# AKASH2907/pi-consistency-activity-detection

Measured on AMD Instinct MI355X. Metric: train clips/sec (bs=8, 16×224×224, I3D+caps+bv cons) at 1/2/4/8 GPU, higher is better.
Workload: dtype f32 (fp32 operands and fp32 accumulation everywhere; 33 of the 79 conv / input-gradient launches and the 3x3x3 / 1x1x1 weight gradients multiply on the bf16 matrix cores: every fp32 operand as the exact sum of 3 bf16 terms, 6 products on v_mfma_f32_32x32x16_bf16, hi / lo fp32 accumulators -- error v

## Files before the change

pi-consistency-activity-detection_amd/csrc/elementwise.hip:

```cpp
#include "common.h"
#include <stdlib.h>

namespace {

constexpr int FIN_RL = 16;
constexpr int FIN_CL = 16;
constexpr int FIN_T = FIN_RL * FIN_CL;

template <typename TP>
__device__ __forceinline__ void partial_colsum(const TP* __restrict__ part, int npg, int C, int c, int rl,
                                               double (*sh)[FIN_RL][FIN_CL], int cl, double& s, double& s2) {
    double a[4] = {0, 0, 0, 0}, b[4] = {0, 0, 0, 0};
    if (c < C) {
        int i = rl;
        for (; i + 3 * FIN_RL < npg; i += 4 * FIN_RL) {
            TP x[4], y[4];
#pragma unroll
            for (int u = 0; u < 4; ++u) { const TP* q = part + (size_t)(i + u * FIN_RL) * 2 * C + c; x[u] = q[0]; y[u] = q[C]; }
#pragma unroll
            for (int u = 0; u < 4; ++u) { a[u] += (double)x[u]; b[u] += (double)y[u]; }
        }
        for (; i < npg; i += FIN_RL) { const TP* q = part + (size_t)i * 2 * C + c; a[0] += (double)q[0]; b[0] += (double)q[C]; }
    }
    sh[0][rl][cl] = (a[0] + a[1]) + (a[2] + a[3]); sh[1][rl][cl] = (b[0] + b[1]) + (b[2] + b[3]);
// ... 525 lines not shown
                if (to > hi[0]) break;
                const int a = t + d.padf[0] - to * ST;
                uchar4 ix[MH * MW];
                f32x4 v[MH * MW];
#pragma unroll
                for (int jh = 0; jh < MH; ++jh)
#pragma unroll
                    for (int jw = 0; jw < MW; ++jw) {
                        const int ho = min(lo[1] + jh, d.Ho - 1), wo = min(lo[2] + jw, d.Wo - 1);
                        const size_t op = (size_t)((n * d.To + to) * d.Ho + ho) * d.Wo + wo;
                        ix[jh * MW + jw] = *(const uchar4*)(am + op * d.C + c);
                        v[jh * MW + jw] = *(const f32x4*)(dy + op * d.ldo + c);
                    }
#pragma unroll
                for (int jh = 0; jh < MH; ++jh)
#pragma unroll
                    for (int jw = 0; jw < MW; ++jw) {
                        const int ho = lo[1] + jh, wo = lo[2] + jw;
                        const int tap = (ho <= hi[1] && wo <= hi[2]) ? (a * KH + (h + d.padf[1] - ho * SH)) * KW + (w + d.padf[2] - wo * SW) : 256;
                        const uchar4 q = ix[jh * MW + jw];
                        const f32x4 u = v[jh * MW + jw];
                        if (q.x == tap) g[0] += u[0];
                        if (q.y == tap) g[1] += u[1];
                        if (q.z == tap) g[2] += u[2];
                        if (q.w == tap) g[3] += u[3];
                    }
            }
        }
        if (accum) g += old;
        *(f32x4*)o = g;
    }
}

__global__ __launch_bounds__(256) void chscale_kernel(const float* __restrict__ x, int ldx, const float* __restrict__ sc, int64_t pos_per_n,
                                                      int C4, int64_t total4, float* __restrict__ y, int ldy, int accum) {
    const int C = C4 * 4;
    for (int64_t idx = (int64_t)blockIdx.x * 256 + threadIdx.x; idx < total4; idx += (int64_t)gridDim.x * 256) {
        const size_t row = (unsigned)idx / (unsigned)C4;
        const int c = (int)((unsigned)idx - (unsigned)row * C4) * 4;
        const size_t n = (unsigned)row / (unsigned)pos_per_n;
        const f32x4 v = *(const f32x4*)(x + row * ldx + c), s = *(const f32x4*)(sc + n * C + c);
        f32x4 o = v * s;
        float* q = y + row * ldy + c;
        if (accum) o += *(const f32x4*)q;
        *(f32x4*)q = o;
    }
}

template <typename T>
__global__ __launch_bounds__(256) void to_ndhwc_kernel(const T* __restrict__ src, int N, int C, int64_t thw, int W, int Cpad, int flipw,
                                                       float* __restrict__ dst) {
    const int64_t total = (int64_t)N * thw;
    for (int64_t idx = (int64_t)blockIdx.x * 256 + threadIdx.x; idx < total; idx += (int64_t)gridDim.x * 256) {
        const int64_t n = idx / thw, pos = idx - n * thw;
        int64_t sp = pos;
        if (flipw) { const int w = (int)(pos % W); sp = pos - w + (W - 1 - w); }
        if (Cpad == 4) {
            f32x4 v;
#pragma unroll
            for (int c = 0; c < 4; ++c) v[c] = c < C ? (float)src[(n * C + c) * thw + sp] : 0.f;
            *(f32x4*)(dst + idx * 4) = v;
            continue;
        }
        for (int c = 0; c < Cpad; ++c)
            dst[idx * Cpad + c] = c < C ? (float)src[(n * C + c) * thw + sp] : 0.f;
    }
// ... 50 lines not shown
        if (i < J.tr) {
            const int r = r0 + i, c = c0 + c4;
            f32x4 sum = {0.f, 0.f, 0.f, 0.f};
            if (r < J.R && c < J.Cc) {
                const f32x4* q = (const f32x4*)(J.src + (size_t)b * J.sbs + (size_t)r * J.sld + c);
                const size_t st4 = (size_t)J.sst / 4;
                int k = 0;
                for (; k + 16 <= J.nsl; k += 16) {
                    f32x4 t[16];
#pragma unroll
                    for (int u = 0; u < 16; ++u) t[u] = q[(size_t)(k + u) * st4];
#pragma unroll
                    for (int u = 0; u < 16; ++u) sum += t[u];
                }
                for (; k + 4 <= J.nsl; k += 4) {
                    f32x4 t[4];
#pragma unroll
                    for (int u = 0; u < 4; ++u) t[u] = q[(size_t)(k + u) * st4];
#pragma unroll
                    for (int u = 0; u < 4; ++u) sum += t[u];
                }
                for (; k < J.nsl; ++k) sum += q[(size_t)k * st4];
            }
            tile[i][c4] = sum[0]; tile[i][c4 + 1] = sum[1]; tile[i][c4 + 2] = sum[2]; tile[i][c4 + 3] = sum[3];
        }
    }
    __syncthreads();
    for (int i = ty; i < 32; i += 8) {
        const int c = c0 + i, r = r0 + tx;
        if (tx < J.tr && c < J.Cc && r < J.R) {
            float* o = J.dst + (size_t)b * J.dbs + (size_t)c * J.dld + r;
            *o = (J.accum ? *o : 0.f) + tile[tx][i];
        }
    }
}

template <int GROUP>
__global__ __launch_bounds__(256) void slices_fold_kernel(float* __restrict__ ws, int64_t image4, int nslices, int64_t total) {
    for (int64_t idx = (int64_t)blockIdx.x * 256 + threadIdx.x; idx < total; idx += (int64_t)gridDim.x * 256) {
        const int64_t e = idx % image4; const int g = (int)(idx / image4);
        float4* base = (float4*)ws + (int64_t)g * GROUP * image4 + e;
        const int n = min(GROUP, nslices - g * GROUP);
        float4 t[GROUP];
#pragma unroll
        for (int k = 0; k < GROUP; ++k) if (k < n) t[k] = base[(int64_t)k * image4];
        float4 sum = t[0];
#pragma unroll
        for (int k = 1; k < GROUP; ++k) if (k < n) { sum.x += t[k].x; sum.y += t[k].y; sum.z += t[k].z; sum.w += t[k].w; }
        base[0] = sum;
    }
}

__global__ __launch_bounds__(256) void fill_kernel(float* p, int64_t n, float v) {
    for (int64_t i = (int64_t)blockIdx.x * 256 + threadIdx.x; i < n; i += (int64_t)gridDim.x * 256) p[i] = v;
}
__global__ __launch_bounds__(256) void axpy_kernel(float* y, const float* x, int64_t n, float a) {
    for (int64_t i = (int64_t)blockIdx.x * 256 + threadIdx.x; i < n; i += (int64_t)gridDim.x * 256) y[i] += a * x[i];
}

__global__ __launch_bounds__(256) void adam_kernel(float* __restrict__ p, const float* __restrict__ g, float* __restrict__ m, float* __restrict__ v,
                                                   int64_t n, float lr_bc1, float b1, float b2, float omb1, float omb2, float eps, float inv_sqrt_bc2,
                                                   float gscale) {
    for (int64_t i = (int64_t)blockIdx.x * 256 + threadIdx.x; i < n; i += (int64_t)gridDim.x * 256) {
        const float gi = g[i] * gscale;
        const float mi = b1 * m[i] + omb1 * gi;
        const float vi = b2 * v[i] + omb2 * gi * gi;
// ... 2 lines not shown
    }
}

__global__ __launch_bounds__(256) void col2im_kernel(const float* __restrict__ cols, int N, int Ho, int Wo, int KH, int KW, int C4,
                                                     float* __restrict__ dx, int lddx, int accum, int64_t total4) {
    const int Hi = Ho + KH - 1, Wi = Wo + KW - 1, C = C4 * 4;
    const size_t ldc = (size_t)KH * KW * C;
    for (int64_t idx = (int64_t)blockIdx.x * 256 + threadIdx.x; idx < total4; idx += (int64_t)gridDim.x * 256) {
        int64_t pos = idx / C4;
        const int c = (int)(idx - pos * C4) * 4;
        const int64_t ipos = pos;
        const int w = (int)(pos % Wi); pos /= Wi;
        const int h = (int)(pos % Hi); const int n = (int)(pos / Hi);
        f32x4 acc = {0.f, 0.f, 0.f, 0.f};
        const int b0 = max(0, h - (Ho - 1)), b1 = min(KH - 1, h), c0 = max(0, w - (Wo - 1)), c1 = min(KW - 1, w);
        for (int b = b0; b <= b1; ++b)
            for (int cc = c0; cc <= c1; ++cc) {
                const size_t op = (size_t)((n * Ho + (h - b)) * Wo + (w - cc));
                acc += *(const f32x4*)(cols + op * ldc + (size_t)(b * KW + cc) * C + c);
            }
        float* o = dx + ipos * lddx + c;
        if (accum) acc += *(const f32x4*)o;
        *(f32x4*)o = acc;
    }
}

inline int grid_for(int64_t n, int per_thread = 1) {
    int64_t b = (n + 256ll * per_thread - 1) / (256ll * per_thread);
    if (b > 256 * 16) b = 256 * 16;
    if (b < 1) b = 1;
    return (int)b;
}
inline int pool_blocks(int64_t total4) { return total4 > POOL_ITEMS ? (int)((total4 + POOL_ITEMS - 1) / POOL_ITEMS) : 1; }
inline int pool_form(const pc_pool_desc* d) {
    const auto is = [](const int32_t* v, int a, int b, int c) { return v[0] == a && v[1] == b && v[2] == c; };
    if (is(d->k, 1, 3, 3) && is(d->s, 1, 2, 2)) return 1;
    if (is(d->k, 3, 3, 3) && is(d->s, 2, 1, 1)) return 2;
    if (is(d->k, 3, 3, 3) && is(d->s, 1, 1, 1)) return 3;
    return 0;
}
inline double pc_decimal_of_float(float x) {
    char buf[40];
    for (int prec = 1; prec <= 9; ++prec) {
        snprintf(buf, sizeof(buf), "%.*g", prec, (double)x);
        const double d = strtod(buf, nullptr);
        if ((float)d == x) return d;
    }
    return (double)x;
}
inline int64_t red_rows_per_block(int64_t rows) {
    int64_t r = (rows + 1023) / 1024;
    if (r < 32) r = 32;
    return r;
}

}

extern "C" int64_t pc_bn_finalize_ws_floats(int nparts_per_group, int groups, int C) {
    return nparts_per_group >= 512 ? (int64_t)groups * FIN_S * 2 * C * 2 + 2 : 0;
}

extern "C" int pc_bn_finalize_ws(const float* part, int nparts_per_group, int groups, int C, int64_t count_per_group,
                                 const float* gamma, const float* beta, float eps, float momentum, float* running_mean,
                                 float* running_var, float* stat, float* ws, pc_stream s) {
    PC_CHECK_ARG(part && gamma && beta && stat && groups >= 1 && C > 0, "pc_bn_finalize: bad args");
    if (ws && nparts_per_group >= 512) {
// ... 80 lines not shown
    {
        RedP p;
        p.a = dy; p.lda = lddy; p.b = z; p.ldb = ldz;
        p.stat = stat; p.C4 = C / 4; p.rows = rpg; p.rows_per_group = rpg; p.rows_per_block = rpb;
        p.act = relu ? PC_ACT_RELU : PC_ACT_NONE; p.part = part;
        p.a_gs = rpg * lddy; p.b_gs = rpg * ldz; p.stat_gs = 4 * C; p.part_gs = (int64_t)npg * 2 * C;
        hipLaunchKernelGGL(colreduce_kernel, dim3(npg, groups), dim3(256), 0, s, p);
    }
    PC_CHECK_LAUNCH("bn_bwd reduce");
    if (fused) {
        PC_CHECK_ARG(rows * (int64_t)(C / 4) < (1ll << 31), "elementwise kernels index with 32 bits");
        const int cblocks = cdiv(C, FA_CB), rb2 = fa_rows_per_block(rpg, cblocks, groups);
        hipLaunchKernelGGL(bn_bwd_fin_apply_kernel, dim3((unsigned)cdiv(rpg, rb2), cblocks, groups), dim3(256), 0, s, part, npg, groups, C, (double)rpg, dy, lddy, z, ldz,
                           stat, relu, dz, lddz, dgamma, dbeta, accum, (int)rpg, rb2);
        PC_CHECK_LAUNCH("bn_bwd fin_apply");
        return PC_OK;
    }
    hipLaunchKernelGGL(bn_bwd_finalize_kernel, dim3(cdiv(C, FIN_CL)), dim3(FIN_T), 0, s, part, npg, groups, C, (double)rpg, coef, dgamma, dbeta, accum);
    const int64_t total4 = rows * (C / 4);
    PC_CHECK_ARG(total4 < (1ll << 31), "elementwise kernels index with 32 bits: %lld float4 elements", (long long)total4);
    hipLaunchKernelGGL(bn_bwd_apply_kernel, dim3(grid_for(total4, 2)), dim3(256), 0, s, dy, lddy, z, ldz, stat, coef, C / 4, total4, rpg, relu, dz, lddz);
    PC_CHECK_LAUNCH("bn_bwd apply");
    return PC_OK;
}

extern "C" int pc_maxpool_fwd(const pc_pool_desc* d, const float* x, float* y, uint8_t* argmax, pc_stream s) {
    PC_CHECK_ARG(d && x && y && argmax && d->C % 4 == 0 && d->ldi % 4 == 0 && d->ldo % 4 == 0, "pc_maxpool_fwd: bad args");
    PC_CHECK_ARG(d->k[0] * d->k[1] * d->k[2] < 255, "pc_maxpool_fwd: window too large");
    const int64_t npos = (int64_t)d->N * d->To * d->Ho * d->Wo, total4 = npos * (d->C / 4);
    PC_CHECK_ARG(total4 < (1ll << 31), "elementwise kernels index with 32 bits: %lld float4 elements", (long long)total4);
    const int nblk = pool_blocks(total4);
    const unsigned ppb = (unsigned)cdiv(npos, nblk);
#define PC_POOL_FWD(...) hipLaunchKernelGGL((maxpool_fwd_kernel<__VA_ARGS__>), dim3(nblk), dim3(256), 0, (hipStream_t)s, *d, x, y, argmax, (unsigned)npos, ppb)
    switch (pool_form(d)) {
        case 1: PC_POOL_FWD(1, 3, 3, 1, 2, 2); break;
        case 2: PC_POOL_FWD(3, 3, 3, 2, 1, 1); break;
        case 3: PC_POOL_FWD(3, 3, 3, 1, 1, 1); break;
        default: PC_POOL_FWD(0, 0, 0, 0, 0, 0);
    }
#undef PC_POOL_FWD
    PC_CHECK_LAUNCH("maxpool_fwd");
    return PC_OK;
}

extern "C" int pc_maxpool_bwd(const pc_pool_desc* d, const float* dy, const uint8_t* argmax, float* dx, int accum, pc_stream s) {
    PC_CHECK_ARG(d && dy && dx && argmax && d->C % 4 == 0 && d->ldi % 4 == 0 && d->ldo % 4 == 0, "pc_maxpool_bwd: bad args");
    const int64_t npos = (int64_t)d->N * d->Ti * d->Hi * d->Wi, total4 = npos * (d->C / 4);
    PC_CHECK_ARG(total4 < (1ll << 31), "elementwise kernels index with 32 bits: %lld float4 elements", (long long)total4);
    const int nblk = pool_blocks(total4);
    const unsigned ppb = (unsigned)cdiv(npos, nblk);
#define PC_POOL_BWD(...) hipLaunchKernelGGL((maxpool_bwd_kernel<__VA_ARGS__>), dim3(nblk), dim3(256), 0, (hipStream_t)s, *d, dy, argmax, dx, accum, (unsigned)npos, ppb)
    switch (pool_form(d)) {
        case 1: PC_POOL_BWD(1, 3, 3, 1, 2, 2); break;
        case 2: PC_POOL_BWD(3, 3, 3, 2, 1, 1); break;
        case 3: PC_POOL_BWD(3, 3, 3, 1, 1, 1); break;
        default: PC_POOL_BWD(0, 0, 0, 0, 0, 0);
    }
#undef PC_POOL_BWD
    PC_CHECK_LAUNCH("maxpool_bwd");
    return PC_OK;
}

extern "C" int pc_channel_scale(const float* x, int ldx, const float* scale, int N, int64_t pos_per_n, int C, float* y, int ldy,
                                int accum, pc_stream s) {
    PC_CHECK_ARG(x && scale && y && C % 4 == 0 && ldx % 4 == 0 && ldy % 4 == 0, "pc_channel_scale: bad args");
    const int64_t total4 = (int64_t)N * pos_per_n * (C / 4);
    PC_CHECK_ARG(total4 < (1ll << 31), "elementwise kernels index with 32 bits: %lld float4 elements", (long long)total4);
    hipLaunchKernelGGL(chscale_kernel, dim3(grid_for(total4, 2)), dim3(256), 0, (hipStream_t)s, x, ldx, scale, pos_per_n, C / 4, total4, y, ldy, accum);
    PC_CHECK_LAUNCH("channel_scale");
    return PC_OK;
}

extern "C" int64_t pc_act_bwd_ws_floats(int64_t rows, int C) {
    const int64_t rpb = red_rows_per_block(rows);
    return ((rows + rpb - 1) / rpb) * 2 * (int64_t)C + 64;
}

extern "C" int pc_act_bwd(const float* dy, int lddy, const float* y, int ldy, int act, int C, int64_t rows, float* dz, int lddz,
                          float* dbias, int accum, float* ws, pc_stream s_) {
    hipStream_t s = (hipStream_t)s_;
    PC_CHECK_ARG(dy && y && C % 4 == 0 && C <= 1024 && lddy % 4 == 0 && ldy % 4 == 0, "pc_act_bwd: bad args (C=%d)", C);
    const bool write = dz && (act != PC_ACT_NONE || dz != dy);
    const int64_t total4 = rows * (C / 4);
    if (write) {
        PC_CHECK_ARG(lddz % 4 == 0, "pc_act_bwd: lddz");
        PC_CHECK_ARG(total4 < (1ll << 31), "elementwise kernels index with 32 bits: %lld float4 elements", (long long)total4);
    }
    if (dbias) {
        PC_CHECK_ARG(ws, "pc_act_bwd: ws required for dbias");
        const int64_t rpb = red_rows_per_block(rows);
// ... 6 lines not shown
    }
    PC_CHECK_LAUNCH("act_bwd");
    return PC_OK;
}

extern "C" int pc_ncdhw_to_ndhwc(const void* src, int src_is_f64, int N, int C, int64_t thw, int W, int Cpad, int flipw, float* dst, pc_stream s) {
    PC_CHECK_ARG(src && dst && Cpad >= C && W > 0 && thw % W == 0, "pc_ncdhw_to_ndhwc: bad args");
    const int64_t total = (int64_t)N * thw;
    if (src_is_f64) hipLaunchKernelGGL(to_ndhwc_kernel<double>, dim3(grid_for(total)), dim3(256), 0, (hipStream_t)s, (const double*)src, N, C, thw, W, Cpad, flipw, dst);
    else hipLaunchKernelGGL(to_ndhwc_kernel<float>, dim3(grid_for(total)), dim3(256), 0, (hipStream_t)s, (const float*)src, N, C, thw, W, Cpad, flipw, dst);
    PC_CHECK_LAUNCH("to_ndhwc");
    return PC_OK;
}

extern "C" int pc_ndhwc_to_ncdhw(const float* src, int ld, int N, int C, int64_t thw, float* dst, pc_stream s) {
    PC_CHECK_ARG(src && dst, "pc_ndhwc_to_ncdhw: null");
    hipLaunchKernelGGL(to_ncdhw_kernel, dim3(grid_for((int64_t)N * C * thw)), dim3(256), 0, (hipStream_t)s, src, ld, N, C, thw, dst);
    PC_CHECK_LAUNCH("to_ncdhw");
    return PC_OK;
}

extern "C" int pc_transpose_batched(const float* src, int batch, int R, int Cc, int64_t src_batch_stride, int src_ld, float* dst,
                                    int64_t dst_batch_stride, int dst_ld, int accum, pc_stream s) {
    PC_CHECK_ARG(src && dst && batch >= 1 && batch <= 65535 && R >= 1 && Cc >= 1, "pc_transpose_batched: bad args");
    PC_CHECK_ARG(cdiv(R, 32) <= 65535, "pc_transpose_batched: too many row tiles");
    hipLaunchKernelGGL(transpose_kernel, dim3(cdiv(Cc, 32), cdiv(R, 32), batch), dim3(256), 0, (hipStream_t)s, src, R, Cc, src_batch_stride,
                       src_ld, dst, dst_batch_stride, dst_ld, accum);
    PC_CHECK_LAUNCH("transpose");
    return PC_OK;
}

extern "C" int pc_transpose_multi(const pc_transpose_job* jobs, int njobs, pc_stream s) {
    PC_CHECK_ARG(jobs && njobs >= 1, "pc_transpose_multi: bad args");
    for (int j0 = 0; j0 < njobs; j0 += TM_JOBS) {
        TPack pk;
        pk.n = njobs - j0 < TM_JOBS ? njobs - j0 : TM_JOBS;
        int tiles = 0;
        for (int q = 0; q < pk.n; ++q) {
            const pc_transpose_job& a = jobs[j0 + q];
            PC_CHECK_ARG(a.src && a.dst && a.batch >= 1 && a.R >= 1 && a.C >= 1, "pc_transpose_multi: bad job %d", j0 + q);
            TJobK& k = pk.j[q];
            k.src = (const float*)(uintptr_t)a.src; k.dst = (float*)(uintptr_t)a.dst; k.sbs = a.src_batch_stride; k.dbs = a.dst_batch_stride;
            PC_CHECK_ARG(a.nslices >= 0 && (a.nslices <= 1 || a.slice_stride > 0), "pc_transpose_multi: job %d has %d slices %lld floats apart", j0 + q, a.nslices, (long long)a.slice_stride);
            k.R = a.R; k.Cc = a.C; k.sld = a.src_ld; k.dld = a.dst_ld; k.accum = a.accum; k.nsl = a.nslices; k.sst = a.slice_stride;
            PC_CHECK_ARG(a.nslices <= 1 || (a.C <= a.src_ld && a.src_ld % 4 == 0 && a.slice_stride % 4 == 0 && a.src_batch_stride % 4 == 0 && a.src % 16 == 0),
                         "pc_transpose_multi: job %d sums slice images: src_ld (>= C) and the strides must be multiples of 4 floats and src 16-byte aligned", j0 + q);
            k.tr = (a.nslices > 1 && (long long)a.batch * cdiv(a.C, 32) * cdiv(a.R, 32) < 192) ? 8 : 32; k.pad_ = 0;
            k.tiles_c = cdiv(a.C, 32); k.tiles_rc = k.tiles_c * cdiv(a.R, k.tr);
            pk.first[q] = tiles;
            tiles += a.batch * k.tiles_rc;
        }
        pk.first[pk.n] = tiles;
        hipLaunchKernelGGL(transpose_multi_kernel, dim3(tiles), dim3(256), 0, (hipStream_t)s, pk);
        PC_CHECK_LAUNCH("transpose_multi");
    }
    return PC_OK;
}

extern "C" int pc_wgrad_fold_group(void) { return 16; }

extern "C" int pc_wgrad_fold(float* ws, int64_t image_floats, int nslices, pc_stream s) {
    PC_CHECK_ARG(ws && image_floats > 0 && image_floats % 4 == 0 && nslices >= 1 && (uintptr_t)ws % 16 == 0, "pc_wgrad_fold: bad args (image %lld floats, %d slices)", (long long)image_floats, nslices);
    constexpr int GROUP = 16;
    if (nslices <= 1) return PC_OK;
    const int64_t total = (image_floats / 4) * cdiv(nslices, GROUP);
    hipLaunchKernelGGL(slices_fold_kernel<GROUP>, dim3(grid_for(total)), dim3(256), 0, (hipStream_t)s, ws, image_floats / 4, nslices, total);
    PC_CHECK_LAUNCH("slices_fold");
    return PC_OK;
}

extern "C" int pc_col2im(const float* cols, int N, int Ho, int Wo, int KH, int KW, int C, float* dx, int lddx, int accum, pc_stream s) {
    PC_CHECK_ARG(cols && dx && C % 4 == 0 && lddx % 4 == 0, "pc_col2im: bad args");
    const int64_t total4 = (int64_t)N * (Ho + KH - 1) * (Wo + KW - 1) * (C / 4);
    hipLaunchKernelGGL(col2im_kernel, dim3(grid_for(total4)), dim3(256), 0, (hipStream_t)s, cols, N, Ho, Wo, KH, KW, C / 4, dx, lddx, accum, total4);
    PC_CHECK_LAUNCH("col2im");
    return PC_OK;
}

extern "C" int pc_fill(float* p, int64_t n, float v, pc_stream s) {
    PC_CHECK_ARG(p || n == 0, "pc_fill: null");
    if (n == 0) return PC_OK;
    hipLaunchKernelGGL(fill_kernel, dim3(grid_for(n, 4)), dim3(256), 0, (hipStream_t)s, p, n, v);
    PC_CHECK_LAUNCH("fill");
    return PC_OK;
}

extern "C" int pc_axpy(float* y, const float* x, int64_t n, float a, pc_stream s) {
    PC_CHECK_ARG((y && x) || n == 0, "pc_axpy: null");
    if (n == 0) return PC_OK;
// ... 17 lines not shown
```

pi-consistency-activity-detection_amd/csrc/tail6.hip:

```cpp
#include "common.h"
#include <stdlib.h>

namespace {

constexpr int NSLOT = 125, SP = 128, J32 = 32;

__device__ __forceinline__ int npairs(int k5, bool first) { return k5 == 0 || k5 == 4 ? 1 : (k5 == 2 ? (first ? 2 : 3) : 2); }
__device__ __forceinline__ int pair_k4(int k5, bool first, int q) {
    switch (k5) {
        case 0: return 0;
        case 1: return q;
        case 2: return first ? 1 + q : q;
        case 3: return 1 + q;
        default: return 2;
    }
}

__global__ __launch_bounds__(256) void tail6_weights_kernel(const float* __restrict__ wf, int N, int Ci, float* __restrict__ W5f,
                                                            float* __restrict__ W5t) {
    const int64_t total = (int64_t)N * 8 * SP * Ci;
    for (int64_t idx = (int64_t)blockIdx.x * 256 + threadIdx.x; idx < total; idx += (int64_t)gridDim.x * 256) {
        const int ci = (int)(idx % Ci);
        const int slot = (int)((idx / Ci) % SP);
        const int z = (int)((idx / ((int64_t)Ci * SP)) % 8);
// ... 95 lines not shown
                const float f = (vt && vh) ? 1.f : 0.f;
                const float* pl = base + (size_t)((kt * 5 + kh) * 5) * P3 + ((size_t)itc * Ih + ihc) * Iw;
                const float e0 = pl[iwp], e2 = pl[2 * P3 + qw], e4 = pl[4 * P3 + iwm];
                const float o1 = pl[P3 + iwp], o3 = pl[3 * P3 + qw];
                acc0 += f * ((fwp * e0 + e2) + fwm * e4);
                acc1 += f * (fwp * o1 + o3);
            }
        }
        float b0, b1;
        const bool w0b = qw == 0, w1b = qw == Iw - 1;
        if (!tb && !hb && !w0b && !w1b) { b0 = b1 = sbc[27]; }
        else {
            b0 = b1 = 0.f;
            for (int a = 0; a < 3; ++a) {
                const int mt = ot + 1 - a;
                if (mt < 0 || mt >= Ot) continue;
                for (int b = 0; b < 3; ++b) {
                    const int mh = oh + 1 - b;
                    if (mh < 0 || mh >= Oh) continue;
                    for (int c = 0; c < 3; ++c) {
                        const int m0 = 2 * qw + 1 - c, m1 = 2 * qw + 2 - c;
                        const float v = sbc[(a * 3 + b) * 3 + c];
                        if (m0 >= 0 && m0 < Ow) b0 += v;
                        if (m1 >= 0 && m1 < Ow) b1 += v;
                    }
                }
            }
        }
        const float bs = bsm[0];
        *(float2*)(out + (((size_t)n * Ot + ot) * Oh + oh) * Ow + 2 * qw) = make_float2(bs + b0 + acc0, bs + b1 + acc1);
    }
}

__global__ __launch_bounds__(256) void tail6_scatter_kernel(const float* __restrict__ dout, int N, int It, int Ih, int Iw, float* __restrict__ dcols) {
    const int Ot = 2 * It, Oh = 2 * Ih, Ow = 2 * Iw;
    const int64_t total = (int64_t)N * It * Ih * Iw * (SP / 4);
    const int64_t idx = (int64_t)blockIdx.x * 256 + threadIdx.x;
    if (idx >= total) return;
    const int q4 = (int)(idx % (SP / 4));
    const int64_t pos = idx / (SP / 4);
    const int iw = (int)(pos % Iw), ih = (int)((pos / Iw) % Ih), it = (int)((pos / ((int64_t)Iw * Ih)) % It), n = (int)(pos / ((int64_t)Iw * Ih * It));
    float v[4];
#pragma unroll
    for (int e = 0; e < 4; ++e) {
        const int slot = q4 * 4 + e;
        v[e] = 0.f;
        if (slot >= NSLOT) continue;
        const int o0 = 2 * it - 2 + slot / 25, o1 = 2 * ih - 2 + (slot / 5) % 5, o2 = 2 * iw - 2 + slot % 5;
        if (o0 >= 0 && o0 < Ot && o1 >= 0 && o1 < Oh && o2 >= 0 && o2 < Ow) v[e] = dout[(((size_t)n * Ot + o0) * Oh + o1) * Ow + o2];
    }
    *(float4*)(dcols + pos * SP + q4 * 4) = make_float4(v[0], v[1], v[2], v[3]);
}

struct T6Slices { int n[8]; long long zoff[8]; long long image; };

__global__ __launch_bounds__(256) void tail6_slices_sum_kernel(float* __restrict__ ws, const T6Slices sl) {
    const int z = blockIdx.y, ns = sl.n[z];
    if (ns < 2) return;
    float4* base = (float4*)(ws + sl.zoff[z]);
    const long long img4 = sl.image / 4;
    for (long long e = (long long)blockIdx.x * 256 + threadIdx.x; e < img4; e += (long long)gridDim.x * 256) {
        float4 v = base[e];
        int k = 1;
        for (; k + 8 <= ns; k += 8) {
            float4 t[8];
#pragma unroll
            for (int u = 0; u < 8; ++u) t[u] = base[(long long)(k + u) * img4 + e];
#pragma unroll
            for (int u = 0; u < 8; ++u) { v.x += t[u].x; v.y += t[u].y; v.z += t[u].z; v.w += t[u].w; }
        }
        for (; k < ns; ++k) { const float4 t = base[(long long)k * img4 + e]; v.x += t.x; v.y += t.y; v.z += t.z; v.w += t.w; }
        base[e] = v;
    }
}
__global__ __launch_bounds__(256) void tail6_wgrad_map_kernel(const float* __restrict__ dW5, int N, int Ci, float* __restrict__ Gc, const T6Slices sl) {
    const int64_t total = (int64_t)N * Ci * 27 * J32;
    for (int64_t idx = (int64_t)blockIdx.x * 256 + threadIdx.x; idx < total; idx += (int64_t)gridDim.x * 256) {
        const int j = (int)(idx & 31);
        const int tap = (int)((idx >> 5) % 27);
        const int ci = (int)((idx / (27 * J32)) % Ci);
        const int n = (int)(idx / ((int64_t)27 * J32 * Ci));
        float acc = 0.f;
        if (j < 27) {
            const int k4[3] = {tap / 9, (tap / 3) % 3, tap % 3}, ks[3] = {j / 9, (j / 3) % 3, j % 3};
// ... 66 lines not shown

}

extern "C" int pc_tail6_weights(const float* wf, int N, int Ci, float* W5f, float* W5t, pc_stream s) {
    PC_CHECK_ARG(wf && W5f && W5t && N >= 1 && Ci >= 1, "pc_tail6_weights: bad args");
    const int64_t total = (int64_t)N * 8 * SP * Ci;
    int grid = (int)((total + 255) / 256); if (grid > 8192) grid = 8192;
    hipLaunchKernelGGL(tail6_weights_kernel, dim3(grid), dim3(256), 0, (hipStream_t)s, wf, N, Ci, W5f, W5t);
    PC_CHECK_LAUNCH("tail6_weights");
    return PC_OK;
}

extern "C" int pc_tail6_gather(const float* cols, const float* bc, const float* bsm, int N, int It, int Ih, int Iw, float* out, pc_stream s) {
    PC_CHECK_ARG(cols && bc && bsm && out && N >= 1 && It >= 1 && Ih >= 1 && Iw >= 1, "pc_tail6_gather: bad args");
    const int64_t total = (int64_t)N * 8 * It * Ih * Iw;
    PC_CHECK_ARG((total + 255) / 256 < (1ll << 31), "pc_tail6_gather: too large");
    if (((uintptr_t)out & 7) == 0) {
        const dim3 grid((unsigned)((int64_t)N * It * Ih));
        hipLaunchKernelGGL((tail6_gather_rows_kernel<0, 0>), grid, dim3(128), 0, (hipStream_t)s, cols, bc, bsm, N, It, Ih, Iw, out);
        hipLaunchKernelGGL((tail6_gather_rows_kernel<0, 1>), grid, dim3(128), 0, (hipStream_t)s, cols, bc, bsm, N, It, Ih, Iw, out);
        hipLaunchKernelGGL((tail6_gather_rows_kernel<1, 0>), grid, dim3(128), 0, (hipStream_t)s, cols, bc, bsm, N, It, Ih, Iw, out);
        hipLaunchKernelGGL((tail6_gather_rows_kernel<1, 1>), grid, dim3(128), 0, (hipStream_t)s, cols, bc, bsm, N, It, Ih, Iw, out);
    } else {
        hipLaunchKernelGGL(tail6_gather_kernel, dim3((unsigned)cdiv(total, 256)), dim3(256), 0, (hipStream_t)s, cols, bc, bsm, N, It, Ih, Iw, out);
    }
    PC_CHECK_LAUNCH("tail6_gather");
    return PC_OK;
}

extern "C" int pc_tail6_scatter(const float* dout, int N, int It, int Ih, int Iw, float* dcols, pc_stream s) {
    PC_CHECK_ARG(dout && dcols && N >= 1 && It >= 1 && Ih >= 1 && Iw >= 1, "pc_tail6_scatter: bad args");
    const int64_t total = (int64_t)N * It * Ih * Iw * (SP / 4);
    PC_CHECK_ARG((total + 255) / 256 < (1ll << 31), "pc_tail6_scatter: too large");
    hipLaunchKernelGGL(tail6_scatter_kernel, dim3((unsigned)cdiv(total, 256)), dim3(256), 0, (hipStream_t)s, dout, N, It, Ih, Iw, dcols);
    PC_CHECK_LAUNCH("tail6_scatter");
    return PC_OK;
}

static int t6_wgrad_map(float* dW5, const int32_t* nslices8, int N, int Ci, float* Gc, pc_stream s) {
    PC_CHECK_ARG(dW5 && Gc && N >= 1 && Ci >= 1, "pc_tail6_wgrad_map: bad args");
    T6Slices sl;
    sl.image = nslices8 ? (long long)N * Ci * SP : 0;
    long long at = 0;
    for (int z = 0; z < 8; ++z) {
        sl.n[z] = nslices8 ? nslices8[z] : 1;
        PC_CHECK_ARG(sl.n[z] >= 0 && sl.n[z] <= 65536, "pc_tail6_wgrad_map_slices: class %d has %d slice images", z, sl.n[z]);
        sl.zoff[z] = at;
        at += sl.n[z] * sl.image;
    }
    const int64_t total = (int64_t)N * Ci * 27 * J32;
    int grid = (int)((total + 255) / 256); if (grid > 8192) grid = 8192;
    if (sl.image) {
        int g4 = (int)((sl.image / 4 + 255) / 256); if (g4 > 512) g4 = 512;
        hipLaunchKernelGGL(tail6_slices_sum_kernel, dim3(g4, 8), dim3(256), 0, (hipStream_t)s, dW5, sl);
    }
    hipLaunchKernelGGL(tail6_wgrad_map_kernel, dim3(grid), dim3(256), 0, (hipStream_t)s, dW5, N, Ci, Gc, sl);
    PC_CHECK_LAUNCH("tail6_wgrad_map");
    return PC_OK;
}

extern "C" int pc_tail6_wgrad_map_slices(float* ws, const int32_t* nslices8, int N, int Ci, float* Gc, pc_stream s) {
    PC_CHECK_ARG(nslices8, "pc_tail6_wgrad_map_slices: no slice counts");
    return t6_wgrad_map(ws, nslices8, N, Ci, Gc, s);
}

extern "C" int pc_tail6_wgrad_map(const float* dW5, int N, int Ci, float* Gc, pc_stream s) {
    return t6_wgrad_map(const_cast<float*>(dW5), nullptr, N, Ci, Gc, s);
// ... 33 lines not shown
```

Before: 446.6.

## Tile 3x3x3 maxpool kernels, add row relayout path, stage tail6 scatter in LDS

Adds register-tiled forward and backward kernels for the 3x3x3 max pools. The forward kernel computes a 2x2 output tile per thread and the backward kernel a strip of four input columns, so neighbouring windows reuse loaded values instead of re-reading them. Transpose jobs that are really row copies or slice sums now go to a separate vectorised row kernel instead of the 32x32 tile transpose. The tail6 scatter first stages a run of dout rows in shared memory, then writes the column buffer from there, cutting redundant global reads. The cost is higher register pressure in the pool kernels and more launch paths to keep correct.

```diff
diff --git a/pi-consistency-activity-detection_amd/csrc/elementwise.hip b/pi-consistency-activity-detection_amd/csrc/elementwise.hip
--- a/pi-consistency-activity-detection_amd/csrc/elementwise.hip
+++ b/pi-consistency-activity-detection_amd/csrc/elementwise.hip
@@ -581,6 +581,152 @@
     }
 }
 
+constexpr int POOL_WT = 4;
+
+template <int ST>
+__global__ __launch_bounds__(256, 4) void maxpool333_fwd_tile_kernel(const pc_pool_desc d, const float* __restrict__ x, float* __restrict__ y,
+                                                                     uint8_t* __restrict__ am, unsigned nitems) {
+    const unsigned C4 = (unsigned)d.C / 4, tw = ((unsigned)d.Wo + 1) / 2, th = ((unsigned)d.Ho + 1) / 2;
+    const unsigned i = (unsigned)xcd_remap((int)blockIdx.x, (int)gridDim.x) * 256 + threadIdx.x;
+    if (i < nitems) {
+        unsigned q = i / C4;
+        const int c = (int)(i % C4) * 4;
+        const int wo0 = (int)(q % tw) * 2; q /= tw;
+        const int ho0 = (int)(q % th) * 2; q /= th;
+        const int to = (int)(q % (unsigned)d.To); const int n = (int)(q / (unsigned)d.To);
+        f32x4 best[4];
+        unsigned bi[4];
+#pragma unroll
+        for (int u = 0; u < 4; ++u) {
+            best[u] = f32x4{-INFINITY, -INFINITY, -INFINITY, -INFINITY};
+            bi[u] = 0xFFFFFFFFu;
+        }
+        const int h0 = ho0 - d.padf[1], w0 = wo0 - d.padf[2];
+#pragma unroll 1
+        for (int a = 0; a < 3; ++a) {
+            const int t = to * ST - d.padf[0] + a;
+            if ((unsigned)t >= (unsigned)d.Ti) {
+#pragma unroll
+                for (int u = 0; u < 4; ++u)
+#pragma unroll
+                    for (int e = 0; e < 4; ++e)
+                        if (0.f > best[u][e]) { best[u][e] = 0.f; bi[u] |= 0xFFu << (8 * e); }
+                continue;
+            }
+            f32x4 v[4][4];
+            const unsigned pb = ((unsigned)((n * d.Ti + t) * d.Hi) * (unsigned)d.Wi * (unsigned)d.ldi + (unsigned)c) * 4u;
+            int h0a = h0, w0a = w0;
+            asm volatile("" : "+v"(h0a), "+v"(w0a));
+#pragma unroll
+            for (int r = 0; r < 4; ++r)
+#pragma unroll
+                for (int j = 0; j < 4; ++j) {
+                    const int h = min(max(h0a + r, 0), d.Hi - 1), w = min(max(w0a + j, 0), d.Wi - 1);
+                    v[r][j] = *(const f32x4*)((const char*)x + (pb + (unsigned)(h * d.Wi + w) * (unsigned)d.ldi * 4u));
+                }
+#pragma unroll
+            for (int r = 0; r < 4; ++r)
+#pragma unroll
+                for (int j = 0; j < 4; ++j)
+                    if (!((unsigned)(h0 + r) < (unsigned)d.Hi && (unsigned)(w0 + j) < (unsigned)d.Wi)) v[r][j] = f32x4{0.f, 0.f, 0.f, 0.f};
+            const unsigned tap0 = (unsigned)a * 9u;
+#pragma unroll
+            for (int u = 0; u < 4; ++u)
+#pragma unroll
+                for (int b = 0; b < 3; ++b)
+#pragma unroll
+                    for (int cc = 0; cc < 3; ++cc) {
+                        const unsigned tap4 = (tap0 + (unsigned)(b * 3 + cc)) * 0x01010101u;
+                        const f32x4 z = v[u / 2 + b][u % 2 + cc];
+#pragma unroll
+                        for (int e = 0; e < 4; ++e) {
+                            const unsigned m = 0xFFu << (8 * e);
+                            if (z[e] > best[u][e]) { best[u][e] = z[e]; bi[u] = (bi[u] & ~m) | (tap4 & m); }
+                        }
+                    }
+        }
+#pragma unroll
+        for (int u = 0; u < 4; ++u) {
+            const int ho = ho0 + u / 2, wo = wo0 + u % 2;
+            unsigned in9 = 0;
+#pragma unroll
+            for (int b = 0; b < 3; ++b)
+#pragma unroll
+                for (int cc = 0; cc < 3; ++cc)
+                    if ((unsigned)(h0 + u / 2 + b) < (unsigned)d.Hi && (unsigned)(w0 + u % 2 + cc) < (unsigned)d.Wi) in9 |= 1u << (b * 3 + cc);
+            const unsigned in27 = in9 | in9 << 9 | in9 << 18;
+#pragma unroll
+            for (int e = 0; e < 4; ++e)
+                if (!(in27 >> ((bi[u] >> (8 * e)) & 31u) & 1u)) bi[u] |= 0xFFu << (8 * e);
+            if (ho < d.Ho && wo < d.Wo) {
+                const size_t opos = (size_t)((n * d.To + to) * d.Ho + ho) * d.Wo + wo;
+                *(f32x4*)(y + opos * d.ldo + c) = best[u];
+                *(unsigned*)(am + opos * d.C + c) = bi[u];
+            }
+        }
+    }
+}
+
+template <int ST, int WT>
+__global__ __launch_bounds__(256, 4) void maxpool333_bwd_tile_kernel(const pc_pool_desc d, const float* __restrict__ dy, const uint8_t* __restrict__ am,
+                                                                     float* __restrict__ dx, int accum, unsigned nitems) {
+    const unsigned C4 = (unsigned)d.C / 4, tw = ((unsigned)d.Wi + WT - 1) / WT;
+    const unsigned i = (unsigned)xcd_remap((int)blockIdx.x, (int)gridDim.x) * 256 + threadIdx.x;
+    if (i < nitems) {
+        unsigned q = i / C4;
+        const int c = (int)(i % C4) * 4;
+        const int w0 = (int)(q % tw) * WT; q /= tw;
+        const int h = (int)(q % (unsigned)d.Hi); q /= (unsigned)d.Hi;
+        const int t = (int)(q % (unsigned)d.Ti); const int n = (int)(q / (unsigned)d.Ti);
+        f32x4 g[WT];
+#pragma unroll
+        for (int u = 0; u < WT; ++u) g[u] = f32x4{0.f, 0.f, 0.f, 0.f};
+        const int top = t + d.padf[0], bot = top - 2;
+        const int thi = min(top / ST, d.To - 1), tlo = bot <= 0 ? 0 : (bot + ST - 1) / ST;
+        const int hb = h + d.padf[1] - 2, wb = w0 + d.padf[2] - 2;
+        constexpr int MT = (3 + ST - 1) / ST;
+#pragma unroll 1
+        for (int jt = 0; jt < MT; ++jt) {
+            const int to = tlo + jt;
+            if (to > thi) break;
+            const int a = top - to * ST;
+            uchar4 ix[3][WT + 2];
+            f32x4 v[3][WT + 2];
+#pragma unroll
+            for (int jh = 0; jh < 3; ++jh)
+#pragma unroll
+                for (int j = 0; j < WT + 2; ++j) {
+                    const int ho = min(max(hb + jh, 0), d.Ho - 1), wo = min(max(wb + j, 0), d.Wo - 1);
+                    const size_t op = (size_t)((n * d.To + to) * d.Ho + ho) * d.Wo + wo;
+                    ix[jh][j] = *(const uchar4*)(am + op * d.C + c);
+                    v[jh][j] = *(const f32x4*)(dy + op * d.ldo + c);
+                }
+#pragma unroll
+            for (int jh = 0; jh < 3; ++jh)
+#pragma unroll
+                for (int u = 0; u < WT; ++u)
+#pragma unroll
+                    for (int jw = 0; jw < 3; ++jw) {
+                        const bool ok = (unsigned)(hb + jh) < (unsigned)d.Ho && (unsigned)(wb + u + jw) < (unsigned)d.Wo;
+                        const int tap = ok ? (a * 3 + (2 - jh)) * 3 + (2 - jw) : 256;
+                        const uchar4 k = ix[jh][u + jw];
+                        const f32x4 z = v[jh][u + jw];
+                        if (k.x == tap) g[u][0] += z[0];
+                        if (k.y == tap) g[u][1] += z[1];
+                        if (k.z == tap) g[u][2] += z[2];
+                        if (k.w == tap) g[u][3] += z[3];
+                    }
+        }
+        float* o = dx + ((size_t)((n * d.Ti + t) * d.Hi + h) * d.Wi + w0) * d.ldi + c;
+#pragma unroll
+        for (int u = 0; u < WT; ++u)
+            if (w0 + u < d.Wi) {
+                if (accum) g[u] += *(const f32x4*)(o + (size_t)u * d.ldi);
+                *(f32x4*)(o + (size_t)u * d.ldi) = g[u];
+            }
+    }
+}
+
 __global__ __launch_bounds__(256) void chscale_kernel(const float* __restrict__ x, int ldx, const float* __restrict__ sc, int64_t pos_per_n,
                                                       int C4, int64_t total4, float* __restrict__ y, int ldy, int accum) {
     const int C = C4 * 4;
@@ -697,6 +843,61 @@
             float* o = J.dst + (size_t)b * J.dbs + (size_t)c * J.dld + r;
             *o = (J.accum ? *o : 0.f) + tile[tx][i];
         }
+    }
+}
+
+struct RJobK { const float* src; float* dst; long long sbs, dbs, sst; int batch, L, dstep, accum, nsl, qpr, vld, vst; };
+struct RPack { RJobK j[TM_JOBS]; int first[TM_JOBS + 1]; int n; };
+
+__global__ __launch_bounds__(256) void relayout_rows_kernel(const RPack pk) {
+    int k = 0;
+    while (k + 1 < pk.n && (int)blockIdx.x >= pk.first[k + 1]) ++k;
+    const RJobK& J = pk.j[k];
+    const long long gq = (long long)((int)blockIdx.x - pk.first[k]) * 256 + threadIdx.x;
+    const long long b = gq / J.qpr;
+    if (b >= J.batch) return;
+    const int c = (int)(gq - b * J.qpr) * 4;
+    const float* s = J.src + b * J.sbs + c;
+    f32x4 v = {0.f, 0.f, 0.f, 0.f};
+    if (J.nsl <= 1) {
+        if (J.vld) v = *(const f32x4*)s;
+        else {
+#pragma unroll
+            for (int e = 0; e < 4; ++e)
+                if (c + e < J.L) v[e] = s[e];
+        }
+    } else {
+        const f32x4* q = (const f32x4*)s;
+        const size_t st4 = (size_t)J.sst / 4;
+        int i = 0;
+        for (; i + 16 <= J.nsl; i += 16) {
+            f32x4 t[16];
+#pragma unroll
+            for (int u = 0; u < 16; ++u) t[u] = q[(size_t)(i + u) * st4];
+#pragma unroll
+            for (int u = 0; u < 16; ++u) v += t[u];
+        }
+        for (; i + 4 <= J.nsl; i += 4) {
+            f32x4 t[4];
+#pragma unroll
+            for (int u = 0; u < 4; ++u) t[u] = q[(size_t)(i + u) * st4];
+#pragma unroll
+            for (int u = 0; u < 4; ++u) v += t[u];
+        }
+        for (; i < J.nsl; ++i) v += q[(size_t)i * st4];
+    }
+    float* o = J.dst + b * J.dbs + (long long)c * J.dstep;
+    if (J.vst && c + 4 <= J.L) {
+        f32x4 old = {0.f, 0.f, 0.f, 0.f};
+        if (J.accum) old = *(const f32x4*)o;
+        *(f32x4*)o = old + v;
+    } else {
+#pragma unroll
+        for (int e = 0; e < 4; ++e)
+            if (c + e < J.L) {
+                float* p = o + (long long)e * J.dstep;
+                *p = (J.accum ? *p : 0.f) + v[e];
+            }
     }
 }
 
@@ -765,6 +966,8 @@
     return (int)b;
 }
 inline int pool_blocks(int64_t total4) { return total4 > POOL_ITEMS ? (int)((total4 + POOL_ITEMS - 1) / POOL_ITEMS) : 1; }
+inline int64_t pool_tile_items(int64_t rows, int W, int C4) { return rows * ((W + POOL_WT - 1) / POOL_WT) * C4; }
+inline bool pool_in_4g(const pc_pool_desc* d) { return (int64_t)d->N * d->Ti * d->Hi * d->Wi * d->ldi * 4 < (1ll << 32); }
 inline int pool_form(const pc_pool_desc* d) {
     const auto is = [](const int32_t* v, int a, int b, int c) { return v[0] == a && v[1] == b && v[2] == c; };
     if (is(d->k, 1, 3, 3) && is(d->s, 1, 2, 2)) return 1;
@@ -911,12 +1114,20 @@
     const int nblk = pool_blocks(total4);
     const unsigned ppb = (unsigned)cdiv(npos, nblk);
 #define PC_POOL_FWD(...) hipLaunchKernelGGL((maxpool_fwd_kernel<__VA_ARGS__>), dim3(nblk), dim3(256), 0, (hipStream_t)s, *d, x, y, argmax, (unsigned)npos, ppb)
+#define PC_POOL_FWD_TILE(ST)                                                                                                                     \
+    do {                                                                                                                                         \
+        const int64_t items = (int64_t)d->N * d->To * ((d->Ho + 1) / 2) * ((d->Wo + 1) / 2) * (d->C / 4);                                       \
+        hipLaunchKernelGGL((maxpool333_fwd_tile_kernel<ST>), dim3(items > 256 ? (unsigned)cdiv(items, 256) : 1), dim3(256), 0, (hipStream_t)s, \
+                           *d, x, y, argmax, (unsigned)items);                                                                                   \
+    } while (0)
+    const bool tile = pool_in_4g(d);
     switch (pool_form(d)) {
         case 1: PC_POOL_FWD(1, 3, 3, 1, 2, 2); break;
-        case 2: PC_POOL_FWD(3, 3, 3, 2, 1, 1); break;
-        case 3: PC_POOL_FWD(3, 3, 3, 1, 1, 1); break;
+        case 2: if (tile) PC_POOL_FWD_TILE(2); else PC_POOL_FWD(3, 3, 3, 2, 1, 1); break;
+        case 3: if (tile) PC_POOL_FWD_TILE(1); else PC_POOL_FWD(3, 3, 3, 1, 1, 1); break;
         default: PC_POOL_FWD(0, 0, 0, 0, 0, 0);
     }
+#undef PC_POOL_FWD_TILE
 #undef PC_POOL_FWD
     PC_CHECK_LAUNCH("maxpool_fwd");
     return PC_OK;
@@ -929,12 +1140,19 @@
     const int nblk = pool_blocks(total4);
     const unsigned ppb = (unsigned)cdiv(npos, nblk);
 #define PC_POOL_BWD(...) hipLaunchKernelGGL((maxpool_bwd_kernel<__VA_ARGS__>), dim3(nblk), dim3(256), 0, (hipStream_t)s, *d, dy, argmax, dx, accum, (unsigned)npos, ppb)
+#define PC_POOL_BWD_TILE(ST)                                                                                                                     \
+    do {                                                                                                                                         \
+        const int64_t items = pool_tile_items((int64_t)d->N * d->Ti * d->Hi, d->Wi, d->C / 4);                                                  \
+        hipLaunchKernelGGL((maxpool333_bwd_tile_kernel<ST, POOL_WT>), dim3(items > 256 ? (unsigned)cdiv(items, 256) : 1), dim3(256), 0, (hipStream_t)s, \
+                           *d, dy, argmax, dx, accum, (unsigned)items);                                                                          \
+    } while (0)
     switch (pool_form(d)) {
         case 1: PC_POOL_BWD(1, 3, 3, 1, 2, 2); break;
-        case 2: PC_POOL_BWD(3, 3, 3, 2, 1, 1); break;
-        case 3: PC_POOL_BWD(3, 3, 3, 1, 1, 1); break;
+        case 2: PC_POOL_BWD_TILE(2); break;
+        case 3: PC_POOL_BWD_TILE(1); break;
         default: PC_POOL_BWD(0, 0, 0, 0, 0, 0);
     }
+#undef PC_POOL_BWD_TILE
 #undef PC_POOL_BWD
     PC_CHECK_LAUNCH("maxpool_bwd");
     return PC_OK;
@@ -1007,29 +1225,74 @@
 
 extern "C" int pc_transpose_multi(const pc_transpose_job* jobs, int njobs, pc_stream s) {
     PC_CHECK_ARG(jobs && njobs >= 1, "pc_transpose_multi: bad args");
-    for (int j0 = 0; j0 < njobs; j0 += TM_JOBS) {
-        TPack pk;
-        pk.n = njobs - j0 < TM_JOBS ? njobs - j0 : TM_JOBS;
-        int tiles = 0;
-        for (int q = 0; q < pk.n; ++q) {
-            const pc_transpose_job& a = jobs[j0 + q];
-            PC_CHECK_ARG(a.src && a.dst && a.batch >= 1 && a.R >= 1 && a.C >= 1, "pc_transpose_multi: bad job %d", j0 + q);
-            TJobK& k = pk.j[q];
-            k.src = (const float*)(uintptr_t)a.src; k.dst = (float*)(uintptr_t)a.dst; k.sbs = a.src_batch_stride; k.dbs = a.dst_batch_stride;
-            PC_CHECK_ARG(a.nslices >= 0 && (a.nslices <= 1 || a.slice_stride > 0), "pc_transpose_multi: job %d has %d slices %lld floats apart", j0 + q, a.nslices, (long long)a.slice_stride);
-            k.R = a.R; k.Cc = a.C; k.sld = a.src_ld; k.dld = a.dst_ld; k.accum = a.accum; k.nsl = a.nslices; k.sst = a.slice_stride;
-            PC_CHECK_ARG(a.nslices <= 1 || (a.C <= a.src_ld && a.src_ld % 4 == 0 && a.slice_stride % 4 == 0 && a.src_batch_stride % 4 == 0 && a.src % 16 == 0),
-                         "pc_transpose_multi: job %d sums slice images: src_ld (>= C) and the strides must be multiples of 4 floats and src 16-byte aligned", j0 + q);
-            k.tr = (a.nslices > 1 && (long long)a.batch * cdiv(a.C, 32) * cdiv(a.R, 32) < 192) ? 8 : 32; k.pad_ = 0;
-            k.tiles_c = cdiv(a.C, 32); k.tiles_rc = k.tiles_c * cdiv(a.R, k.tr);
-            pk.first[q] = tiles;
-            tiles += a.batch * k.tiles_rc;
-        }
+    for (int j = 0; j < njobs; ++j) {
+        const pc_transpose_job& a = jobs[j];
+        PC_CHECK_ARG(a.src && a.dst && a.batch >= 1 && a.R >= 1 && a.C >= 1, "pc_transpose_multi: bad job %d", j);
+        PC_CHECK_ARG(a.nslices >= 0 && (a.nslices <= 1 || a.slice_stride > 0), "pc_transpose_multi: job %d has %d slices %lld floats apart", j, a.nslices, (long long)a.slice_stride);
+        PC_CHECK_ARG(a.nslices <= 1 || (a.C <= a.src_ld && a.src_ld % 4 == 0 && a.slice_stride % 4 == 0 && a.src_batch_stride % 4 == 0 && a.src % 16 == 0),
+                     "pc_transpose_multi: job %d sums slice images: src_ld (>= C) and the strides must be multiples of 4 floats and src 16-byte aligned", j);
+    }
+    const auto is_rows = [](const pc_transpose_job& a) { return a.R == 1 || (a.C == 1 && a.src_ld == 1 && a.nslices <= 1); };
+    TPack pk;
+    pk.n = 0;
+    int tiles = 0;
+    const auto flush_tiles = [&]() -> int {
+        if (!pk.n) return PC_OK;
         pk.first[pk.n] = tiles;
         hipLaunchKernelGGL(transpose_multi_kernel, dim3(tiles), dim3(256), 0, (hipStream_t)s, pk);
         PC_CHECK_LAUNCH("transpose_multi");
-    }
-    return PC_OK;
+        pk.n = 0; tiles = 0;
+        return PC_OK;
+    };
+    for (int j = 0; j < njobs; ++j) {
+        const pc_transpose_job& a = jobs[j];
+        if (is_rows(a)) continue;
+        TJobK k;
+        k.src = (const float*)(uintptr_t)a.src; k.dst = (float*)(uintptr_t)a.dst; k.sbs = a.src_batch_stride; k.dbs = a.dst_batch_stride;
+        k.R = a.R; k.Cc = a.C; k.sld = a.src_ld; k.dld = a.dst_ld; k.accum = a.accum; k.nsl = a.nslices; k.sst = a.slice_stride;
+        k.tr = (a.nslices > 1 && (long long)a.batch * cdiv(a.C, 32) * cdiv(a.R, 32) < 192) ? 8 : 32; k.pad_ = 0;
+        k.tiles_c = cdiv(a.C, 32); k.tiles_rc = k.tiles_c * cdiv(a.R, k.tr);
+        const long long t = (long long)a.batch * k.tiles_rc;
+        PC_CHECK_ARG(t < (1ll << 30), "pc_transpose_multi: job %d is too large", j);
+        if (tiles + t >= (1ll << 30)) { const int rc = flush_tiles(); if (rc != PC_OK) return rc; }
+        pk.j[pk.n] = k;
+        pk.first[pk.n++] = tiles;
+        tiles += (int)t;
+        if (pk.n == TM_JOBS) { const int rc = flush_tiles(); if (rc != PC_OK) return rc; }
+    }
+    { const int rc = flush_tiles(); if (rc != PC_OK) return rc; }
+    RPack rp;
+    rp.n = 0;
+    int units = 0;
+    const auto flush_rows = [&]() -> int {
+        if (!rp.n) return PC_OK;
+        rp.first[rp.n] = units;
+        hipLaunchKernelGGL(relayout_rows_kernel, dim3(units), dim3(256), 0, (hipStream_t)s, rp);
+        PC_CHECK_LAUNCH("transpose_multi rows");
+        rp.n = 0; units = 0;
+        return PC_OK;
+    };
+    for (int j = 0; j < njobs; ++j) {
+        const pc_transpose_job& a = jobs[j];
+        if (!is_rows(a)) continue;
+        RJobK k;
+        k.src = (const float*)(uintptr_t)a.src; k.dst = (float*)(uintptr_t)a.dst; k.sbs = a.src_batch_stride; k.dbs = a.dst_batch_stride; k.sst = a.slice_stride;
+        k.batch = a.batch; k.accum = a.accum; k.nsl = a.nslices;
+        if (a.R == 1) { k.L = a.C; k.dstep = a.dst_ld; }
+        else { k.L = a.R; k.dstep = 1; }
+        k.qpr = cdiv(k.L, 4);
+        const bool rows_al = a.batch == 1 || (a.src_batch_stride % 4 == 0);
+        k.vld = a.nslices > 1 || (a.src % 16 == 0 && rows_al && k.L % 4 == 0);
+        k.vst = k.dstep == 1 && a.dst % 16 == 0 && (a.batch == 1 || a.dst_batch_stride % 4 == 0);
+        const long long u = ((long long)a.batch * k.qpr + 255) / 256;
+        PC_CHECK_ARG(u < (1ll << 30), "pc_transpose_multi: job %d is too large", j);
+        if (units + u >= (1ll << 30)) { const int rc = flush_rows(); if (rc != PC_OK) return rc; }
+        rp.j[rp.n] = k;
+        rp.first[rp.n++] = units;
+        units += (int)u;
+        if (rp.n == TM_JOBS) { const int rc = flush_rows(); if (rc != PC_OK) return rc; }
+    }
+    return flush_rows();
 }
 
 extern "C" int pc_wgrad_fold_group(void) { return 16; }
diff --git a/pi-consistency-activity-detection_amd/csrc/tail6.hip b/pi-consistency-activity-detection_amd/csrc/tail6.hip
--- a/pi-consistency-activity-detection_amd/csrc/tail6.hip
+++ b/pi-consistency-activity-detection_amd/csrc/tail6.hip
@@ -151,24 +151,41 @@
     }
 }
 
+constexpr int SC_RUN = 28, SC_LW = 2 * SC_RUN + 3, SC_ZERO = 25 * SC_LW;
 __global__ __launch_bounds__(256) void tail6_scatter_kernel(const float* __restrict__ dout, int N, int It, int Ih, int Iw, float* __restrict__ dcols) {
+    __shared__ float sd[SC_ZERO + 1];
     const int Ot = 2 * It, Oh = 2 * Ih, Ow = 2 * Iw;
-    const int64_t total = (int64_t)N * It * Ih * Iw * (SP / 4);
-    const int64_t idx = (int64_t)blockIdx.x * 256 + threadIdx.x;
-    if (idx >= total) return;
-    const int q4 = (int)(idx % (SP / 4));
-    const int64_t pos = idx / (SP / 4);
-    const int iw = (int)(pos % Iw), ih = (int)((pos / Iw) % Ih), it = (int)((pos / ((int64_t)Iw * Ih)) % It), n = (int)(pos / ((int64_t)Iw * Ih * It));
-    float v[4];
+    const int runs = (Iw + SC_RUN - 1) / SC_RUN;
+    int row = blockIdx.x;
+    const int iw0 = (row % runs) * SC_RUN; row /= runs;
+    const int ih = row % Ih; row /= Ih;
+    const int it = row % It; const int n = row / It;
+    const int ow0 = 2 * iw0 - 2;
+    for (int i = threadIdx.x; i <= SC_ZERO; i += 256) {
+        const int r = i / SC_LW, ow = ow0 + i % SC_LW;
+        const int ot = 2 * it - 2 + r / 5, oh = 2 * ih - 2 + r % 5;
+        float v = 0.f;
+        if (r < 25 && ot >= 0 && ot < Ot && oh >= 0 && oh < Oh && ow >= 0 && ow < Ow) v = dout[(((size_t)n * Ot + ot) * Oh + oh) * Ow + ow];
+        sd[i] = v;
+    }
+    const int q4 = threadIdx.x & (SP / 4 - 1);
+    int off[4];
 #pragma unroll
     for (int e = 0; e < 4; ++e) {
         const int slot = q4 * 4 + e;
-        v[e] = 0.f;
-        if (slot >= NSLOT) continue;
-        const int o0 = 2 * it - 2 + slot / 25, o1 = 2 * ih - 2 + (slot / 5) % 5, o2 = 2 * iw - 2 + slot % 5;
-        if (o0 >= 0 && o0 < Ot && o1 >= 0 && o1 < Oh && o2 >= 0 && o2 < Ow) v[e] = dout[(((size_t)n * Ot + o0) * Oh + o1) * Ow + o2];
-    }
-    *(float4*)(dcols + pos * SP + q4 * 4) = make_float4(v[0], v[1], v[2], v[3]);
+        off[e] = slot < NSLOT ? (slot / 5) * SC_LW + slot % 5 : SC_ZERO;
+    }
+    __syncthreads();
+    const int nl = min(SC_RUN, Iw - iw0);
+    float* out = dcols + ((((size_t)n * It + it) * Ih + ih) * Iw + iw0) * SP + q4 * 4;
+#pragma unroll
+    for (int l = threadIdx.x / (SP / 4); l < SC_RUN; l += 256 / (SP / 4)) {
+        if (l >= nl) break;
+        float v[4];
+#pragma unroll
+        for (int e = 0; e < 4; ++e) v[e] = sd[off[e] < SC_ZERO ? off[e] + 2 * l : SC_ZERO];
+        *(float4*)(out + (size_t)l * SP) = make_float4(v[0], v[1], v[2], v[3]);
+    }
 }
 
 struct T6Slices { int n[8]; long long zoff[8]; long long image; };
@@ -301,7 +318,9 @@
     PC_CHECK_ARG(dout && dcols && N >= 1 && It >= 1 && Ih >= 1 && Iw >= 1, "pc_tail6_scatter: bad args");
     const int64_t total = (int64_t)N * It * Ih * Iw * (SP / 4);
     PC_CHECK_ARG((total + 255) / 256 < (1ll << 31), "pc_tail6_scatter: too large");
-    hipLaunchKernelGGL(tail6_scatter_kernel, dim3((unsigned)cdiv(total, 256)), dim3(256), 0, (hipStream_t)s, dout, N, It, Ih, Iw, dcols);
+    const int64_t nblk = (int64_t)N * It * Ih * cdiv(Iw, SC_RUN);
+    PC_CHECK_ARG(nblk < (1ll << 31), "pc_tail6_scatter: too large");
+    hipLaunchKernelGGL(tail6_scatter_kernel, dim3((unsigned)nblk), dim3(256), 0, (hipStream_t)s, dout, N, It, Ih, Iw, dcols);
     PC_CHECK_LAUNCH("tail6_scatter");
     return PC_OK;
 }
```

Result: faster. 452.8, median of 6 (+1.4%).
